# Niccolo-Ajroldi/plainLM

Measured on AMD Instinct MI355X. Metric: tokens/sec fwd+bwd (160M, seq=1024, bf16), higher is better.
Workload: dtype bf16

## Files before the change

plainlm_amd/csrc/attn_causal.hip:

```cpp
#include "plm_device.h"

#include <type_traits>

#include "attn_common.h"

template <int RB>
__device__ __forceinline__ void attn_block2(int T, int nh, int& tile, int& h, int& b) {
  const int ntile = (T + RB - 1) / RB;
  const int nbh = gridDim.x / ntile;
  const int bh = blockIdx.x % nbh;
  tile = blockIdx.x / nbh;
  h = bh % nh;
  b = bh / nh;
}

constexpr int ATTN_DMA_PER_STAGE = 4;
constexpr int ATTN_DMA_STATS = 2;
static_assert(ATTN_DMA_PER_STAGE == 2 * 2, "stage() = two TileDma::issue calls of two instructions each");

#define ATTN_DEFER_LOG2 8.0f
#define PLM_ATTN_TRACE_SETTER plm_dbg_attn_trace_causal
ATTN_TRACE_DECL()
#ifdef PLM_ATTN_ONEPASS_ABLATION
static __device__ float* g_onepass_buf = nullptr;
// ... 68 lines not shown
  f32x16_t o[2][2];
  float mc[2], lsum[2];
#pragma unroll
  for (int qb = 0; qb < 2; ++qb) {
    zero16(o[qb][0]);
    zero16(o[qb][1]);
    mc[qb] = -INFINITY;
    lsum[qb] = 0.f;
  }

  auto soft_pv = [&](int qb_, f32x16_t (&s)[2], const bf16x8_t (&vfr)[2][4], int kv0, auto mask_tag) {
    constexpr bool MASK = decltype(mask_tag)::value;
    const int qb = qb_;
    const int c_hi = r0[qb] + l31 - kv0 - 4 * hi;
    float tmax = -INFINITY;
#pragma unroll
    for (int kb = 0; kb < 2; ++kb)
#pragma unroll
      for (int r = 0; r < 16; ++r) {
        if (MASK) {
          const int c = kb * 32 + (r & 3) + 8 * (r >> 2);
          if (c > c_hi) s[kb][r] = -INFINITY;
        }
        tmax = fmaxf(tmax, s[kb][r]);
      }
    {
      float t_lo, t_hi;
      half_pair(tmax, t_lo, t_hi);
      tmax = fmaxf(t_lo, t_hi);
    }
    const float tm = tmax * c2;
    const bool need = tm > mc[qb] + ATTN_DEFER_LOG2;
    if (__builtin_amdgcn_ballot_w64(need) != 0ull) {
      const float mn = fmaxf(mc[qb], tm);
      const float alpha = fast_exp2(mc[qb] - ((mn == -INFINITY) ? 0.f : mn));
      mc[qb] = mn;
      lsum[qb] *= alpha;
#pragma unroll
      for (int db = 0; db < 2; ++db)
#pragma unroll
        for (int r = 0; r < 16; ++r) o[qb][db][r] *= alpha;
    }
    const float mref = (MASK && mc[qb] == -INFINITY) ? 0.f : mc[qb];
    float ps[4] = {0.f, 0.f, 0.f, 0.f};
    bf16x8_t pf[4];
#pragma unroll
    for (int kb = 0; kb < 2; ++kb)
#pragma unroll
      for (int r = 0; r < 16; ++r) {
        const float p = fast_exp2(__builtin_fmaf(s[kb][r], c2, -mref));
        ps[r & 3] += p;
        pf[kb * 2 + (r >> 3)][r & 7] = f2bf(p);
      }
    lsum[qb] += (ps[0] + ps[1]) + (ps[2] + ps[3]);
#pragma unroll
    for (int db = 0; db < 2; ++db)
#pragma unroll
      for (int sp = 0; sp < 4; ++sp) o[qb][db] = mfma32(vfr[db][sp], pf[sp], o[qb][db]);
  };

  auto compute = [&](int kv0, const char* sK, const char* sV, auto m0_tag, auto m1_tag) {
    constexpr int M0 = decltype(m0_tag)::value, M1 = decltype(m1_tag)::value;
    bf16x8_t kfr[2][4];
#pragma unroll
    for (int kb = 0; kb < 2; ++kb)
#pragma unroll
      for (int ks = 0; ks < 4; ++ks) kfr[kb][ks] = frag_rows(sK, kb * 32 + l31, ks, hi);
    f32x16_t s[2][2];
#pragma unroll
    for (int qb = 0; qb < 2; ++qb) {
      if ((qb == 0 ? M0 : M1) == QB_OFF) continue;
#pragma unroll
      for (int kb = 0; kb < 2; ++kb) {
        zero16(s[qb][kb]);
#pragma unroll
        for (int ks = 0; ks < 4; ++ks) s[qb][kb] = mfma32(kfr[kb][ks], qf[qb][ks], s[qb][kb]);
      }
    }
    __builtin_amdgcn_sched_barrier(0);
    bf16x8_t vfr[2][4];
#pragma unroll
    for (int db = 0; db < 2; ++db)
#pragma unroll
      for (int sp = 0; sp < 4; ++sp) vfr[db][sp] = frag_cols(sV, db, (sp >> 1) * 32 + (sp & 1) * 16 + 4 * hi, lane);
    if (M0 == QB_UM) soft_pv(0, s[0], vfr, kv0, std::false_type{});
    if (M0 == QB_MASK) soft_pv(0, s[0], vfr, kv0, std::true_type{});
    if (M1 == QB_UM) soft_pv(1, s[1], vfr, kv0, std::false_type{});
    if (M1 == QB_MASK) soft_pv(1, s[1], vfr, kv0, std::true_type{});
  };

  int i = 0, slot = 0;
  auto run = [&](int jt_end, auto m0_tag, auto m1_tag, bool active) {
    for (; jt_lo + i < jt_end; ++i) {
      const int rem = min(NST - 2, n - 1 - i);
      if (NST >= 4 && rem >= 2) attn_wait_vm<2 * ATTN_DMA_PER_STAGE>();
      else if (NST >= 3 && rem == 1) attn_wait_vm<ATTN_DMA_PER_STAGE>();
      else attn_wait_vm<0>();
      attn_barrier();
      if (i + NST - 1 < n) stage(slot == 0 ? NST - 1 : slot - 1, jt_lo + i + NST - 1);
      if (active) compute((jt_lo + i) * KT, smem + slot * 2 * TILE, smem + slot * 2 * TILE + TILE, m0_tag, m1_tag);
      slot = (slot + 1 == NST) ? 0 : slot + 1;
    }
  };
  using OFF_ = std::integral_constant<int, QB_OFF>;
  using UM_ = std::integral_constant<int, QB_UM>;
  using MK_ = std::integral_constant<int, QB_MASK>;
  const int a0 = min(jt_hi, r0[0] / KT), e0 = min(jt_hi, r0[0] / KT + 1);
  const int a1 = min(jt_hi, r0[1] / KT), e1 = min(jt_hi, r0[1] / KT + 1);
  run(a0, UM_{}, UM_{}, true);
  run(e0, MK_{}, UM_{}, true);
  run(a1, OFF_{}, UM_{}, true);
  run(e1, OFF_{}, MK_{}, true);
  run(jt_hi, OFF_{}, OFF_{}, false);

  const RowStage rs{smem + (n % NST) * 2 * TILE + wave * 4096, lane};
#pragma unroll
  for (int qb = 0; qb < 2; ++qb) {
    const int qrow = r0[qb] + l31;
    float l_lo, l_hi;
    half_pair(lsum[qb], l_lo, l_hi);
    const float ltot = l_lo + l_hi;
    const float inv = 1.f / ltot;
#pragma unroll
    for (int db = 0; db < 2; ++db)
#pragma unroll
      for (int g = 0; g < 4; ++g) {
        bf16x4_t v;
#pragma unroll
        for (int e = 0; e < 4; ++e) v[e] = f2bf(o[qb][db][4 * g + e] * inv);
        rs.put(l31, hi, db * 4 + g, v);
      }
    if (qrow < T && hi == 0) lse[((int64_t)b * nh + h) * T + qrow] = mc[qb] + __builtin_amdgcn_logf(ltot);
    rs.flush(out + (int64_t)b * T * dm, dm, r0[qb], T, h * HD);
  }
}

template <int NST>
__global__ __launch_bounds__(256, 2) void attn_bwd_dq_causal_kernel(const uint16_t* __restrict__ qkv, const uint16_t* __restrict__ out,
                                                              const uint16_t* __restrict__ dout, const float* __restrict__ lse,
                                                              float* __restrict__ delta, const float* __restrict__ rcos,
                                                              const float* __restrict__ rsin, uint16_t* __restrict__ dqkv, int T, int nh,
                                                              float dsign) {
  constexpr int KT = 64;
  constexpr int TILE = KT * 128;
  constexpr int QB = 256;
  __shared__ __attribute__((aligned(1024))) char smem[NST * 2 * TILE];

  int tile_, h, b;
  attn_block2<QB>(T, nh, tile_, h, b);
  const int qt = (T + QB - 1) / QB - 1 - tile_;
  const int dm = nh * HD, ld = 3 * dm;
  const int t = threadIdx.x, lane = t & 63;
  const int wave = __builtin_amdgcn_readfirstlane(t >> 6);
  const int l31 = lane & 31, hi = lane >> 5;
  const int q0 = qt * QB;
  const int r0[2] = {q0 + 32 * wave, q0 + 32 * (7 - wave)};
  const uint16_t* base = qkv + (int64_t)b * T * ld + h * HD;
  const float scale = 0.125f, c2 = scale * LOG2E;

  const int kv_hi = min(T, q0 + QB);
  const int jt_hi = (kv_hi + KT - 1) / KT;
  constexpr int jt_lo = 0;
  const int n = jt_hi;

  TileDma dma;
  dma.init(wave, lane, ld);
  auto stage = [&](int slot, int jt) {
    const int kv0 = jt * KT;
    const uint16_t* src = base + (int64_t)kv0 * ld;
    if (kv0 + KT <= T) {
      dma.issue_full(smem + slot * 2 * TILE, src + dm, wave);
      dma.issue_full(smem + slot * 2 * TILE + TILE, src + 2 * dm, wave);
    } else {
      dma.issue(smem + slot * 2 * TILE, src + dm, ld, T - 1 - kv0, wave);
      dma.issue(smem + slot * 2 * TILE + TILE, src + 2 * dm, ld, T - 1 - kv0, wave);
    }
  };

  if (n > 0) stage(0, jt_lo);

  bf16x8_t qf[2][4], dof[2][4];
  float Lq[2], Dq[2];
#pragma unroll
  for (int qb = 0; qb < 2; ++qb) {
    const int qrow = r0[qb] + l31;
    const bool qvalid = qrow < T;
#pragma unroll
    for (int ks = 0; ks < 4; ++ks) {
      const int d0 = ks * 16 + hi * 8;
      qf[qb][ks] = qvalid ? ld_bf16x8(base + (int64_t)qrow * ld + d0) : zero_bf16x8();
      dof[qb][ks] = qvalid ? ld_bf16x8(dout + ((int64_t)b * T + qrow) * dm + h * HD + d0) : zero_bf16x8();
    }
    Lq[qb] = 0.f;
    float part = 0.f;
    if (qvalid) {
      Lq[qb] = lse[((int64_t)b * nh + h) * T + qrow];
#pragma unroll
      for (int ks = 0; ks < 4; ++ks) {
        const bf16x8_t o8 = ld_bf16x8(out + ((int64_t)b * T + qrow) * dm + h * HD + ks * 16 + hi * 8);
#pragma unroll
        for (int e = 0; e < 8; ++e) part += bf2f(o8[e]) * bf2f(dof[qb][ks][e]);
      }
    }
    float d_lo, d_hi;
    half_pair(part, d_lo, d_hi);
    Dq[qb] = d_lo + d_hi;
  }
#pragma unroll
  for (int qb = 0; qb < 2; ++qb)
    asm volatile("; q/dO fragments resident" ::"v"(qf[qb][0]), "v"(qf[qb][1]), "v"(qf[qb][2]), "v"(qf[qb][3]), "v"(dof[qb][0]), "v"(dof[qb][1]),
                 "v"(dof[qb][2]), "v"(dof[qb][3]), "v"(Lq[qb]), "v"(Dq[qb]));
  asm volatile("s_waitcnt vmcnt(0)" ::: "memory");
#pragma unroll
  for (int i = 1; i < NST - 1; ++i)
    if (i < n) stage(i, jt_lo + i);

  f32x16_t dq[2][2];
#pragma unroll
  for (int qb = 0; qb < 2; ++qb) {
    zero16(dq[qb][0]);
    zero16(dq[qb][1]);
  }

  auto block = [&](int qb_, int kb, const bf16x8_t (&kfr)[4], const bf16x8_t (&vfr)[4], const bf16x8_t (&ktr)[2][2], int kv0, auto mask_tag) {
    constexpr bool MASK = decltype(mask_tag)::value;
    const int qb = qb_;
    const int c_hi = r0[qb] + l31 - kv0 - 4 * hi;
    f32x16_t s, dp;
    zero16(s);
    zero16(dp);
#pragma unroll
    for (int ks = 0; ks < 4; ++ks) {
      s = mfma32(kfr[ks], qf[qb][ks], s);
      dp = mfma32(vfr[ks], dof[qb][ks], dp);
    }
    bf16x8_t dsf[2];
#pragma unroll
    for (int r = 0; r < 16; ++r) {
      float p = fast_exp2(__builtin_fmaf(s[r], c2, -Lq[qb]));
      if (MASK) {
        const int c = kb * 32 + (r & 3) + 8 * (r >> 2);
        p = (c <= c_hi) ? p : 0.f;
      }
      dsf[r >> 3][r & 7] = f2bf(p * (dp[r] - Dq[qb]));
    }
#pragma unroll
    for (int s2 = 0; s2 < 2; ++s2)
#pragma unroll
      for (int db = 0; db < 2; ++db) dq[qb][db] = mfma32(ktr[db][s2], dsf[s2], dq[qb][db]);
  };

  auto compute = [&](int kv0, const char* sK, const char* sV, auto m0_tag, auto m1_tag) {
    constexpr int M0 = decltype(m0_tag)::value, M1 = decltype(m1_tag)::value;
#pragma unroll
    for (int kb = 0; kb < 2; ++kb) {
      __builtin_amdgcn_sched_barrier(0);
      bf16x8_t kfr[4], vfr[4], ktr[2][2];
#pragma unroll
      for (int ks = 0; ks < 4; ++ks) {
        kfr[ks] = frag_rows(sK, kb * 32 + l31, ks, hi);
        vfr[ks] = frag_rows(sV, kb * 32 + l31, ks, hi);
      }
#pragma unroll
      for (int s2 = 0; s2 < 2; ++s2)
#pragma unroll
        for (int db = 0; db < 2; ++db) ktr[db][s2] = frag_cols(sK, db, kb * 32 + s2 * 16 + 4 * hi, lane);
      if (M0 == QB_UM) block(0, kb, kfr, vfr, ktr, kv0, std::false_type{});
      if (M0 == QB_MASK) block(0, kb, kfr, vfr, ktr, kv0, std::true_type{});
      if (M1 == QB_UM) block(1, kb, kfr, vfr, ktr, kv0, std::false_type{});
      if (M1 == QB_MASK) block(1, kb, kfr, vfr, ktr, kv0, std::true_type{});
    }
  };

  int i = 0, slot = 0;
  auto run = [&](int jt_end, auto m0_tag, auto m1_tag, bool active) {
    for (; jt_lo + i < jt_end; ++i) {
      const int rem = min(NST - 2, n - 1 - i);
      if (NST >= 4 && rem >= 2) attn_wait_vm<2 * ATTN_DMA_PER_STAGE>();
      else if (NST >= 3 && rem == 1) attn_wait_vm<ATTN_DMA_PER_STAGE>();
      else attn_wait_vm<0>();
      attn_barrier();
      if (i + NST - 1 < n) stage(slot == 0 ? NST - 1 : slot - 1, jt_lo + i + NST - 1);
      if (active) compute((jt_lo + i) * KT, smem + slot * 2 * TILE, smem + slot * 2 * TILE + TILE, m0_tag, m1_tag);
      slot = (slot + 1 == NST) ? 0 : slot + 1;
    }
  };
  using OFF_ = std::integral_constant<int, QB_OFF>;
  using UM_ = std::integral_constant<int, QB_UM>;
  using MK_ = std::integral_constant<int, QB_MASK>;
  const int a0 = min(jt_hi, r0[0] / KT), e0 = min(jt_hi, r0[0] / KT + 1);
  const int a1 = min(jt_hi, r0[1] / KT), e1 = min(jt_hi, r0[1] / KT + 1);
  run(a0, UM_{}, UM_{}, true);
  run(e0, MK_{}, UM_{}, true);
  run(a1, OFF_{}, UM_{}, true);
  run(e1, OFF_{}, MK_{}, true);
  run(jt_hi, OFF_{}, OFF_{}, false);

  const RowStage rs{smem + (n % NST) * 2 * TILE + wave * 4096, lane};
#pragma unroll
  for (int qb = 0; qb < 2; ++qb) {
    if (r0[qb] + l31 < T && hi == 0) delta[((int64_t)b * nh + h) * T + r0[qb] + l31] = Dq[qb] * dsign;
#pragma unroll
    for (int db = 0; db < 2; ++db)
#pragma unroll
      for (int g = 0; g < 4; ++g) {
        bf16x4_t ov;
#pragma unroll
        for (int e = 0; e < 4; ++e) ov[e] = f2bf(dq[qb][db][4 * g + e] * scale);
        rs.put(l31, hi, db * 4 + g, ov);
      }
    rs.flush_rot(dqkv + (int64_t)b * T * ld, ld, r0[qb], T, h * HD, rcos, rsin);
  }
}

template <int NST, bool DOC>
__device__ __forceinline__ void attn_bwd_dkdv_body(char* smem, const uint16_t* __restrict__ qkv, const uint16_t* __restrict__ dout,
                                                   const float* __restrict__ lse, const float* __restrict__ ndelta,
                                                   const float* __restrict__ rcos, const float* __restrict__ rsin,
                                                   const int32_t* __restrict__ doc_end, uint16_t* __restrict__ dqkv, int T, int nh, int b, int h,
                                                   int kv0, int jq_plan, unsigned long long* trace_t = nullptr) {
  constexpr int QT = 64;
  constexpr int TILE = QT * 128;
  constexpr int STAGE = 2 * TILE + 512;
  constexpr int NQB = 2;
  const int dm = nh * HD, ld = 3 * dm;
  const int t = threadIdx.x, lane = t & 63;
  const int wave = __builtin_amdgcn_readfirstlane(t >> 6);
  const int l31 = lane & 31, hi = lane >> 5;
  constexpr int qoff = 0;
  const int kvw0 = kv0 + 32 * wave;
  const int kvrow = kvw0 + l31;
  const bool kvalid = kvrow < T;
  const uint16_t* base = qkv + (int64_t)b * T * ld + h * HD;
  const uint16_t* dobase = dout + (int64_t)b * T * dm + h * HD;
  const float* lrow = lse + ((int64_t)b * nh + h) * T;
  const float* drow = ndelta + ((int64_t)b * nh + h) * T;
  const float scale = 0.125f, c2 = scale * LOG2E;

  const int nqt = (T + QT - 1) / QT;
  const int jq_lo = kv0 / QT;
  const int jq_hi = DOC ? jq_plan : nqt;
  const int n = jq_hi - jq_lo;

  TileDma dma, dmad;
  dma.init(wave, lane, ld);
  dmad.init(wave, lane, dm);
  auto stage = [&](int slot, int jq) {
    const int qt0 = jq * QT;
    char* dst = smem + slot * STAGE;
    if (qt0 + QT <= T) {
      dma.issue_full(dst, base + (int64_t)qt0 * ld, wave);
      dmad.issue_full(dst + TILE, dobase + (int64_t)qt0 * dm, wave);
    } else {
      dma.issue(dst, base + (int64_t)qt0 * ld, ld, T - 1 - qt0, wave);
      dma.issue(dst + TILE, dobase + (int64_t)qt0 * dm, dm, T - 1 - qt0, wave);
    }
    if (wave == 0 && lane < 16) {
      const int q = min(qt0 + lane * 4, T - 4);
      dma16_asm(lrow + q, dst + 2 * TILE);
      dma16_asm(drow + q, dst + 2 * TILE + 256);
    }
  };
  bf16x8_t kf[4], vf[4];
  int de = T;
  if (DOC) {
    static_assert(!DOC || NST == 3, "the prologue parks the wave's rows in slots 1 and 2");
    if (n > 0) stage(0, jq_lo);
    char* kreg = smem + 1 * STAGE + wave * 4096;
    char* vreg = smem + 2 * STAGE + wave * 4096;
    rows_dma(kreg, base + dm, ld, kvw0, T - 1, lane);
    rows_dma(vreg, base + 2 * dm, ld, kvw0, T - 1, lane);
    de = doc_end[(int64_t)b * T + min(kvrow, T - 1)];
    asm volatile("; row data requested" ::"v"(de));
    asm volatile("s_waitcnt vmcnt(0)" ::: "memory");
#pragma unroll
    for (int ks = 0; ks < 4; ++ks) {
      kf[ks] = rows_frag(kreg, l31, ks, hi);
      vf[ks] = rows_frag(vreg, l31, ks, hi);
    }
    attn_barrier();
    if (n > 1) stage(1, jq_lo + 1);
  } else {
#pragma unroll
    for (int i = 0; i < NST - 1; ++i)
      if (i < n) stage(i, jq_lo + i);
#pragma unroll
    for (int ks = 0; ks < 4; ++ks) {
      const uint16_t* p = base + (int64_t)kvrow * ld + ks * 16 + hi * 8;
      kf[ks] = kvalid ? ld_bf16x8(p + dm) : zero_bf16x8();
      vf[ks] = kvalid ? ld_bf16x8(p + 2 * dm) : zero_bf16x8();
    }
    asm volatile("; k/v fragments resident" ::"v"(kf[0]), "v"(kf[1]), "v"(kf[2]), "v"(kf[3]), "v"(vf[0]), "v"(vf[1]), "v"(vf[2]), "v"(vf[3]));
    asm volatile("s_waitcnt vmcnt(0)" ::: "memory");
  }
  const int de_lo = DOC ? __builtin_amdgcn_readlane(de, 0) : T, de_hi = DOC ? __builtin_amdgcn_readlane(de, 31) : T;

  f32x16_t dk[2], dv[2];
  zero16(dk[0]); zero16(dk[1]); zero16(dv[0]); zero16(dv[1]);

  auto compute = [&](int qt0, const char* sQ, auto mask_tag) {
    constexpr bool MASK = decltype(mask_tag)::value;
    const char* sDO = sQ + TILE;
    const float* sL = reinterpret_cast<const float*>(sQ + 2 * TILE);
    const float* sD = sL + 64;
    const int c_lo = kvrow - qt0 - qoff - 4 * hi, c_end = de - qt0 - qoff - 4 * hi;
#pragma unroll
    for (int qb = 0; qb < NQB; ++qb) {
      __builtin_amdgcn_sched_barrier(0);
      if (MASK && qt0 + qoff + qb * 32 + 31 < kvw0) continue;
      if (DOC && MASK && qt0 + qoff + qb * 32 >= de_hi) continue;
      bf16x8_t qfr[4], dofr[4], dotr[2][2], qtr[2][2];
#pragma unroll
      for (int ks = 0; ks < 4; ++ks) {
        qfr[ks] = frag_rows(sQ, qoff + qb * 32 + l31, ks, hi);
        dofr[ks] = frag_rows(sDO, qoff + qb * 32 + l31, ks, hi);
      }
      f32x4_t L4[4];
      f32x16_t s, dp;
#pragma unroll
      for (int g = 0; g < 4; ++g) {
        const int ql0 = qoff + qb * 32 + 8 * g + 4 * hi;
        L4[g] = *reinterpret_cast<const f32x4_t*>(sL + ql0);
        const f32x4_t nd = *reinterpret_cast<const f32x4_t*>(sD + ql0);
#pragma unroll
        for (int e = 0; e < 4; ++e) dp[4 * g + e] = nd[e];
      }
#pragma unroll
      for (int s2 = 0; s2 < 2; ++s2)
#pragma unroll
        for (int db = 0; db < 2; ++db) {
          dotr[db][s2] = frag_cols(sDO, db, qoff + qb * 32 + s2 * 16 + 4 * hi, lane);
          qtr[db][s2] = frag_cols(sQ, db, qoff + qb * 32 + s2 * 16 + 4 * hi, lane);
        }
      zero16(s);
#pragma unroll
      for (int ks = 0; ks < 4; ++ks) {
        s = mfma32(qfr[ks], kf[ks], s);
        dp = mfma32(dofr[ks], vf[ks], dp);
      }
      bf16x8_t pf[2], dsf[2];
#pragma unroll
      for (int g = 0; g < 4; ++g)
#pragma unroll
        for (int e = 0; e < 4; ++e) {
          const int r = 4 * g + e;
          float p = fast_exp2(__builtin_fmaf(s[r], c2, -L4[g][e]));
          if (MASK) {
            const int c = qb * 32 + 8 * g + e;
            p = ((c >= c_lo) && (c < c_end)) ? p : 0.f;
          }
          const float dsv = p * dp[r];
          pf[r >> 3][r & 7] = f2bf(p);
          dsf[r >> 3][r & 7] = f2bf(dsv);
        }
#pragma unroll
      for (int s2 = 0; s2 < 2; ++s2)
#pragma unroll
        for (int db = 0; db < 2; ++db) {
          dv[db] = mfma32(dotr[db][s2], pf[s2], dv[db]);
          dk[db] = mfma32(qtr[db][s2], dsf[s2], dk[db]);
        }
#ifdef PLM_ATTN_ONEPASS_ABLATION
      if (g_onepass_mode) {
        char* scr = smem + NST * STAGE + wave * 2048;
        *reinterpret_cast<bf16x8_t*>(scr + lane * 32) = dsf[0];
        *reinterpret_cast<bf16x8_t*>(scr + lane * 32 + 16) = dsf[1];
        bf16x8_t at[2];
#pragma unroll
        for (int s2 = 0; s2 < 2; ++s2)
          at[s2] = join_tr(lds_read_tr16(scr + s2 * 1024 + (lane & 15) * 64 + (lane >> 4) * 8), lds_read_tr16(scr + s2 * 1024 + 512 + (lane & 15) * 32 + (lane >> 4) * 8));
        f32x16_t dqp[2];
        zero16(dqp[0]);
        zero16(dqp[1]);
#pragma unroll
        for (int s2 = 0; s2 < 2; ++s2)
#pragma unroll
          for (int db = 0; db < 2; ++db) dqp[db] = mfma32(at[s2], frag_cols(sQ, db, qoff + qb * 32 + s2 * 16 + 4 * hi, lane), dqp[db]);
        if (g_onepass_mode == 2) {
#pragma unroll
          for (int db = 0; db < 2; ++db)
#pragma unroll
            for (int r = 0; r < 16; ++r) {
              const int q = min(qt0 + qb * 32 + mfma32_row(r, hi), T - 1);
              atomicAdd(g_onepass_buf + ((int64_t)b * T + q) * dm + h * HD + db * 32 + l31, dqp[db][r]);
            }
        } else {
          asm volatile("; partial dQ" ::"v"(dqp[0]), "v"(dqp[1]));
        }
      }
#endif
    }
  };

  const bool wave_rows = kvw0 < T;
  const int jq_act = wave_rows ? min(jq_hi, max(jq_lo, kvw0 / QT)) : jq_hi;
  const int jq_m = min(jq_hi, max(jq_act, (kvw0 + 31 + QT - 1) / QT));
  const int jq_u = min(jq_hi, max(jq_m, de_lo / QT));
  const int jq_e = min(jq_hi, max(jq_u, (de_hi + QT - 1) / QT));
#ifdef PLM_ATTN_TRACE
  if (trace_t) trace_t[0] = __builtin_amdgcn_s_memrealtime();
#endif
  int i = 0, slot = 0;
  auto run = [&](int jq_end, auto mask_tag, bool active) {
    for (; jq_lo + i < jq_end; ++i) {
      const int rem = min(NST - 2, n - 1 - i);
      constexpr int W0 = ATTN_DMA_PER_STAGE + ATTN_DMA_STATS;
      if (wave == 0) {
        if (NST >= 4 && rem >= 2) attn_wait_vm<2 * W0>();
        else if (NST >= 3 && rem == 1) attn_wait_vm<W0>();
        else attn_wait_vm<0>();
      } else {
        if (NST >= 4 && rem >= 2) attn_wait_vm<2 * ATTN_DMA_PER_STAGE>();
        else if (NST >= 3 && rem == 1) attn_wait_vm<ATTN_DMA_PER_STAGE>();
        else attn_wait_vm<0>();
      }
      attn_barrier();
      if (i + NST - 1 < n) stage(slot == 0 ? NST - 1 : slot - 1, jq_lo + i + NST - 1);
      if (active) compute((jq_lo + i) * QT, smem + slot * STAGE, mask_tag);
      slot = (slot + 1 == NST) ? 0 : slot + 1;
    }
  };
  run(jq_act, std::true_type{}, false);
  run(jq_m, std::true_type{}, true);
  run(jq_u, std::false_type{}, true);
  run(jq_e, std::true_type{}, true);
  if (DOC) run(jq_hi, std::true_type{}, false);
#ifdef PLM_ATTN_TRACE
  if (trace_t) trace_t[1] = __builtin_amdgcn_s_memrealtime();
#endif

  const RowStage rs{smem + (n % NST) * STAGE + wave * 4096, lane};
#pragma unroll
  for (int db = 0; db < 2; ++db)
#pragma unroll
    for (int g = 0; g < 4; ++g) {
      bf16x4_t ov;
#pragma unroll
      for (int e = 0; e < 4; ++e) ov[e] = f2bf(dv[db][4 * g + e]);
      rs.put(l31, hi, db * 4 + g, ov);
    }
  rs.flush(dqkv + (int64_t)b * T * ld, ld, kvw0, T, 2 * dm + h * HD);
#pragma unroll
  for (int db = 0; db < 2; ++db)
#pragma unroll
    for (int g = 0; g < 4; ++g) {
      bf16x4_t ok;
#pragma unroll
      for (int e = 0; e < 4; ++e) ok[e] = f2bf(dk[db][4 * g + e] * scale);
      rs.put(l31, hi, db * 4 + g, ok);
    }
  rs.flush_rot(dqkv + (int64_t)b * T * ld, ld, kvw0, T, dm + h * HD, rcos, rsin);
}


template <int NST>
__global__ __launch_bounds__(256, 2) void attn_bwd_dkdv_causal_kernel(const uint16_t* __restrict__ qkv, const uint16_t* __restrict__ dout,
                                                                      const float* __restrict__ lse, const float* __restrict__ ndelta,
                                                                      const float* __restrict__ rcos, const float* __restrict__ rsin,
                                                                      uint16_t* __restrict__ dqkv, int T, int nh) {
  __shared__ __attribute__((aligned(1024))) char smem[NST * (2 * 8192 + 512) + ONEPASS_LDS];
  int kt, h, b;
  attn_block2<128>(T, nh, kt, h, b);
  attn_bwd_dkdv_body<NST, false>(smem, qkv, dout, lse, ndelta, rcos, rsin, nullptr, dqkv, T, nh, b, h, kt * 128, 0);
}

template <int NST>
__global__ __launch_bounds__(256, 2) void attn_bwd_dkdv_doc_kernel(const uint16_t* __restrict__ qkv, const uint16_t* __restrict__ dout,
                                                                   const float* __restrict__ lse, const float* __restrict__ ndelta,
                                                                   const float* __restrict__ rcos, const float* __restrict__ rsin,
                                                                   const int32_t* __restrict__ header, const int32_t* __restrict__ doc_end,
                                                                   const int4* __restrict__ items, uint16_t* __restrict__ dqkv, int T, int nh) {
  __shared__ __attribute__((aligned(1024))) char smem[NST * (2 * 8192 + 512) + ONEPASS_LDS];
  ATTN_TRACE_T(tr0);
  const int idx = blockIdx.x / nh, h = blockIdx.x - idx * nh;
  if (idx >= __builtin_amdgcn_readfirstlane(header[0])) return;
  const int4 it = items[idx];
  const int b = __builtin_amdgcn_readfirstlane(it.x), kv0 = __builtin_amdgcn_readfirstlane(it.y), jq_hi = __builtin_amdgcn_readfirstlane(it.z);
  const int kc = __builtin_amdgcn_readfirstlane(it.w);
  (void)kc;
#ifdef PLM_ATTN_TRACE
  unsigned long long tt[2] = {0, 0};
#else
  unsigned long long* tt = nullptr;
#endif
  attn_bwd_dkdv_body<NST, true>(smem, qkv, dout, lse, ndelta, rcos, rsin, doc_end, dqkv, T, nh, b, h, kv0, jq_hi, tt);
  ATTN_TRACE_END(2, idx, kc, tr0, tt[0], tt[1]);
}

void plm_attn_fwd_causal(const uint16_t* qkv, uint16_t* out, float* lse, int64_t B, int64_t T, int64_t nh, hipStream_t s) {
  const dim3 grid((unsigned)(plm_cdiv(T, 256) * nh * B)), block(256);
  hipLaunchKernelGGL((attn_fwd_causal_kernel<4>), grid, block, 0, s, qkv, out, lse, (int)T, (int)nh);
}
void plm_attn_bwd_causal(const uint16_t* qkv, const uint16_t* out, const uint16_t* dout, const float* lse, float* delta, const float* rc,
                         const float* rs, uint16_t* dqkv, int64_t B, int64_t T, int64_t nh, hipStream_t s) {
  const dim3 block(256);
  hipLaunchKernelGGL((attn_bwd_dq_causal_kernel<3>), dim3((unsigned)(plm_cdiv(T, 256) * nh * B)), block, 0, s, qkv, out, dout, lse, delta, rc, rs, dqkv, (int)T, (int)nh, -1.f);
  hipLaunchKernelGGL((attn_bwd_dkdv_causal_kernel<3>), dim3((unsigned)(plm_cdiv(T, 128) * nh * B)), block, 0, s, qkv, dout, lse, delta, rc, rs, dqkv,
                     (int)T, (int)nh);
}
void plm_attn_bwd_dkdv_doc(const uint16_t* qkv, const uint16_t* dout, const float* lse, const float* ndelta, const float* rc, const float* rs,
                           const int32_t* header, const int32_t* doc_end, const int4* items_k, uint16_t* dqkv, int64_t B, int64_t T, int64_t nh,
                           hipStream_t s) {
  hipLaunchKernelGGL((attn_bwd_dkdv_doc_kernel<3>), dim3((unsigned)(doc_plan_cap(B, T) * nh)), dim3(256), 0, s, qkv, dout, lse, ndelta, rc, rs,
                     header, doc_end, items_k, dqkv, (int)T, (int)nh);
}
```

plainlm_amd/csrc/attn_common.h:

```cpp
#pragma once
#include "plm_device.h"

#define HD 64
#define LOG2E 1.4426950408889634f

__device__ __forceinline__ float fast_exp2(float x) { return __builtin_amdgcn_exp2f(x); }

__device__ __forceinline__ int rs_off(int row, int c) {
  const int pp = ((c >> 1) + 2 * ((row >> 1) & 1) + ((row >> 3) & 1)) & 3;
  const int ph = (c & 1) ^ ((row >> 2) & 1);
  return row * 128 + pp * 32 + ph * 16;
}
__device__ __forceinline__ int rs_logical_chunk(int row, int pc) {
  const int cb = ((pc >> 1) - 2 * ((row >> 1) & 1) - ((row >> 3) & 1)) & 3;
  return cb * 2 + ((pc & 1) ^ ((row >> 2) & 1));
}

__device__ __forceinline__ bf16x8_t frag_rows(const char* tile, int row, int ks, int hi) {
  return *reinterpret_cast<const bf16x8_t*>(tile + rs_off(row, ks * 2 + hi));
}
__device__ __forceinline__ bf16x8_t frag_cols(const char* tile, int db, int rbase, int lane) {
  const int ib = (lane >> 4) & 1, t16 = lane & 15;
  const int sub = t16 & 3;
  const int c = (db * 2 + ib) * 2 + (sub >> 1);
  const int row = rbase + (t16 >> 2);
  const char* p0 = tile + rs_off(row, c) + (sub & 1) * 8;
  const char* p1 = tile + rs_off(row + 8, c) + (sub & 1) * 8;
  return join_tr(lds_read_tr16(p0), lds_read_tr16(p1));
}

struct TileDma {
  int row[2], coff[2];
  unsigned boff[2];
  __device__ __forceinline__ void init(int wave, int lane, int64_t ld = 0) {
#pragma unroll
    for (int i = 0; i < 2; ++i) {
      row[i] = (i * 4 + wave) * 8 + (lane >> 3);
      coff[i] = rs_logical_chunk(row[i], lane & 7) * 8;
      boff[i] = (unsigned)((row[i] * ld + coff[i]) * 2);
    }
  }
  __device__ __forceinline__ void issue(char* dst_tile, const uint16_t* src, int64_t ld, int last_row, int wave, int row0 = 0) const {
#pragma unroll
    for (int i = 0; i < 2; ++i)
      dma16_asm(src + (int64_t)min(row0 + row[i], last_row) * ld + coff[i], dst_tile + (i * 4 + wave) * 1024);
  }
  __device__ __forceinline__ void issue_full(char* dst_tile, const uint16_t* src, int wave) const {
#pragma unroll
    for (int i = 0; i < 2; ++i) dma16_saddr_asm(src, boff[i], dst_tile + (i * 4 + wave) * 1024);
  }
};

__device__ __forceinline__ void rows_dma(char* region, const uint16_t* src, int64_t ld, int row0, int last_row, int lane) {
#pragma unroll
  for (int i = 0; i < 4; ++i) {
    const int row = 8 * i + (lane >> 3);
    dma16_asm(src + (int64_t)min(row0 + row, last_row) * ld + rs_logical_chunk(row, lane & 7) * 8, region + i * 1024);
  }
}
__device__ __forceinline__ bf16x8_t rows_frag(const char* region, int l31, int ks, int hi) {
  return *reinterpret_cast<const bf16x8_t*>(region + rs_off(l31, ks * 2 + hi));
}

template <int N>
__device__ __forceinline__ void attn_wait_vm() {
  asm volatile("s_waitcnt vmcnt(%0)" ::"n"(N) : "memory");
}
__device__ __forceinline__ void attn_barrier() { asm volatile("s_waitcnt lgkmcnt(0)\n\ts_barrier" ::: "memory"); }

__device__ __forceinline__ void zero16(f32x16_t& v) {
#pragma unroll
  for (int r = 0; r < 16; ++r) v[r] = 0.f;
}

struct RowStage {
  char* base;
  int lane;
  __device__ __forceinline__ void put(int l31, int hi, int c16, bf16x4_t v) const {
    *reinterpret_cast<bf16x4_t*>(base + l31 * 128 + ((c16 ^ (l31 & 7)) << 4) + hi * 8) = v;
  }
  __device__ __forceinline__ void flush(uint16_t* dst, int64_t ld, int row0, int row_end, int col0) const {
#pragma unroll
    for (int i = 0; i < 4; ++i) {
      const int row = 8 * i + (lane >> 3), c16 = lane & 7;
      const bf16x8_t v = *reinterpret_cast<const bf16x8_t*>(base + row * 128 + ((c16 ^ (row & 7)) << 4));
      if (row0 + row < row_end) st_bf16x8(dst + (int64_t)(row0 + row) * ld + col0 + c16 * 8, v);
    }
  }
  __device__ __forceinline__ void flush_rot(uint16_t* dst, int64_t ld, int row0, int row_end, int col0, const float* __restrict__ rcos,
                                            const float* __restrict__ rsin) const {
    f32x4_t cs[4], sn[4];
#pragma unroll
    for (int i = 0; i < 4; ++i) {
      const int trow = min(row0 + 8 * i + (lane >> 3), row_end - 1);
      cs[i] = *reinterpret_cast<const f32x4_t*>(rcos + trow * (HD / 2) + (lane & 7) * 4);
      sn[i] = *reinterpret_cast<const f32x4_t*>(rsin + trow * (HD / 2) + (lane & 7) * 4);
    }
#pragma unroll
    for (int i = 0; i < 4; ++i) {
      const int row = 8 * i + (lane >> 3), c16 = lane & 7;
      const bf16x8_t v = *reinterpret_cast<const bf16x8_t*>(base + row * 128 + ((c16 ^ (row & 7)) << 4));
      if (row0 + row < row_end) st_bf16x8(dst + (int64_t)(row0 + row) * ld + col0 + c16 * 8, rope8(v, cs[i], sn[i], -1.f));
    }
  }
};


struct DocPlan {
  const int32_t* header;
  const int32_t* doc_end;
  const int4* items_q;
  const int4* items_k;
};
constexpr int DOC_KIND_SHIFT = 30;
__host__ __device__ __forceinline__ int64_t doc_plan_tiles(int64_t B, int64_t T) { return B * ((T + 127) / 128); }
__host__ __device__ __forceinline__ int64_t doc_plan_cap(int64_t B, int64_t T) { return doc_plan_tiles(B, T) + doc_plan_tiles(B, T) / 4; }
__host__ __device__ __forceinline__ int64_t doc_plan_pq(int64_t B, int64_t T) { return (8 + B * T + 3) & ~(int64_t)3; }
__host__ __device__ __forceinline__ int64_t doc_plan_ints(int64_t B, int64_t T) { return doc_plan_pq(B, T) + 8 * doc_plan_cap(B, T); }
__host__ __device__ __forceinline__ DocPlan doc_plan_view(const int32_t* plan, int64_t B, int64_t T) {
  DocPlan p;
  p.header = plan;
  p.doc_end = plan + 8;
  p.items_q = reinterpret_cast<const int4*>(plan + doc_plan_pq(B, T));
  p.items_k = p.items_q + doc_plan_cap(B, T);
  return p;
}

#ifdef PLM_ATTN_TRACE
#define ATTN_TRACE_DECL()                                                                    \
  static __device__ unsigned long long* g_attn_trace = nullptr;                               \
  extern "C" int PLM_ATTN_TRACE_SETTER(unsigned long long* buf) {                             \
    return (int)hipMemcpyToSymbol(HIP_SYMBOL(g_attn_trace), &buf, sizeof(buf));               \
  }
#define ATTN_TRACE_T(var) const unsigned long long var = __builtin_amdgcn_s_memrealtime()
#define ATTN_TRACE_END(kid, rank_, cost_, t0, t1, t2)                                                                              \
  if (threadIdx.x == 0 && g_attn_trace) {                                                                                          \
    unsigned long long* r_ = g_attn_trace + ((size_t)(kid) * 65536 + blockIdx.x) * 8;                                             \
    r_[0] = t0; r_[1] = t1; r_[2] = t2; r_[3] = __builtin_amdgcn_s_memrealtime();                                                 \
    r_[4] = __builtin_amdgcn_s_getreg((31 << 11) | 4); r_[5] = __builtin_amdgcn_s_getreg((31 << 11) | 20);                         \
    r_[6] = (unsigned long long)(rank_); r_[7] = (unsigned long long)(cost_);                                                      \
  }
#else
#define ATTN_TRACE_DECL()
#define ATTN_TRACE_T(var)
#define ATTN_TRACE_END(kid, rank_, cost_, t0, t1, t2)
#endif
```

Before: 1.053 million.

## Switch causal attention backward kernels from 32x32 to 16x16 MFMA tiles

Rewrites the dQ and dK/dV causal backward kernels to use 16x16x32 MFMA fragments instead of 32x32 ones, with new LDS fragment loaders and a permlane-based row reduction. The finer granularity lets diagonal-masked blocks skip fully masked 16-row sub-blocks, split by wave parity so half the key block is skipped per wave. This trades fewer wasted MFMAs on the causal diagonal for more instructions and fragment loads per useful FLOP and a different register layout.

```diff
diff --git a/plainlm_amd/csrc/attn_causal.hip b/plainlm_amd/csrc/attn_causal.hip
--- a/plainlm_amd/csrc/attn_causal.hip
+++ b/plainlm_amd/csrc/attn_causal.hip
@@ -244,7 +244,6 @@
   const int dm = nh * HD, ld = 3 * dm;
   const int t = threadIdx.x, lane = t & 63;
   const int wave = __builtin_amdgcn_readfirstlane(t >> 6);
-  const int l31 = lane & 31, hi = lane >> 5;
   const int q0 = qt * QB;
   const int r0[2] = {q0 + 32 * wave, q0 + 32 * (7 - wave)};
   const uint16_t* base = qkv + (int64_t)b * T * ld + h * HD;
@@ -271,100 +270,119 @@
 
   if (n > 0) stage(0, jt_lo);
 
-  bf16x8_t qf[2][4], dof[2][4];
-  float Lq[2], Dq[2];
-#pragma unroll
-  for (int qb = 0; qb < 2; ++qb) {
-    const int qrow = r0[qb] + l31;
+  const int l15 = lane & 15, lg = lane >> 4;
+  bf16x8_t qf[4][2], dof[4][2];
+  float Lq[4], Dq[4];
+#pragma unroll
+  for (int j = 0; j < 4; ++j) {
+    const int qrow = r0[j >> 1] + 16 * (j & 1) + l15;
     const bool qvalid = qrow < T;
 #pragma unroll
-    for (int ks = 0; ks < 4; ++ks) {
-      const int d0 = ks * 16 + hi * 8;
-      qf[qb][ks] = qvalid ? ld_bf16x8(base + (int64_t)qrow * ld + d0) : zero_bf16x8();
-      dof[qb][ks] = qvalid ? ld_bf16x8(dout + ((int64_t)b * T + qrow) * dm + h * HD + d0) : zero_bf16x8();
-    }
-    Lq[qb] = 0.f;
+    for (int kk = 0; kk < 2; ++kk) {
+      const int d0 = kchunk16(kk, lg) * 8;
+      qf[j][kk] = qvalid ? ld_bf16x8(base + (int64_t)qrow * ld + d0) : zero_bf16x8();
+      dof[j][kk] = qvalid ? ld_bf16x8(dout + ((int64_t)b * T + qrow) * dm + h * HD + d0) : zero_bf16x8();
+    }
+    Lq[j] = 0.f;
     float part = 0.f;
     if (qvalid) {
-      Lq[qb] = lse[((int64_t)b * nh + h) * T + qrow];
-#pragma unroll
-      for (int ks = 0; ks < 4; ++ks) {
-        const bf16x8_t o8 = ld_bf16x8(out + ((int64_t)b * T + qrow) * dm + h * HD + ks * 16 + hi * 8);
-#pragma unroll
-        for (int e = 0; e < 8; ++e) part += bf2f(o8[e]) * bf2f(dof[qb][ks][e]);
-      }
-    }
-    float d_lo, d_hi;
-    half_pair(part, d_lo, d_hi);
-    Dq[qb] = d_lo + d_hi;
+      Lq[j] = lse[((int64_t)b * nh + h) * T + qrow];
+#pragma unroll
+      for (int kk = 0; kk < 2; ++kk) {
+        const bf16x8_t o8 = ld_bf16x8(out + ((int64_t)b * T + qrow) * dm + h * HD + kchunk16(kk, lg) * 8);
+#pragma unroll
+        for (int e = 0; e < 8; ++e) part += bf2f(o8[e]) * bf2f(dof[j][kk][e]);
+      }
+    }
+    Dq[j] = sum_groups16(part);
   }
 #pragma unroll
-  for (int qb = 0; qb < 2; ++qb)
-    asm volatile("; q/dO fragments resident" ::"v"(qf[qb][0]), "v"(qf[qb][1]), "v"(qf[qb][2]), "v"(qf[qb][3]), "v"(dof[qb][0]), "v"(dof[qb][1]),
-                 "v"(dof[qb][2]), "v"(dof[qb][3]), "v"(Lq[qb]), "v"(Dq[qb]));
+  for (int j = 0; j < 4; ++j)
+    asm volatile("; q/dO fragments resident" ::"v"(qf[j][0]), "v"(qf[j][1]), "v"(dof[j][0]), "v"(dof[j][1]), "v"(Lq[j]), "v"(Dq[j]));
   asm volatile("s_waitcnt vmcnt(0)" ::: "memory");
 #pragma unroll
   for (int i = 1; i < NST - 1; ++i)
     if (i < n) stage(i, jt_lo + i);
 
-  f32x16_t dq[2][2];
-#pragma unroll
-  for (int qb = 0; qb < 2; ++qb) {
-    zero16(dq[qb][0]);
-    zero16(dq[qb][1]);
-  }
-
-  auto block = [&](int qb_, int kb, const bf16x8_t (&kfr)[4], const bf16x8_t (&vfr)[4], const bf16x8_t (&ktr)[2][2], int kv0, auto mask_tag) {
-    constexpr bool MASK = decltype(mask_tag)::value;
-    const int qb = qb_;
-    const int c_hi = r0[qb] + l31 - kv0 - 4 * hi;
-    f32x16_t s, dp;
-    zero16(s);
-    zero16(dp);
-#pragma unroll
-    for (int ks = 0; ks < 4; ++ks) {
-      s = mfma32(kfr[ks], qf[qb][ks], s);
-      dp = mfma32(vfr[ks], dof[qb][ks], dp);
-    }
-    bf16x8_t dsf[2];
-#pragma unroll
-    for (int r = 0; r < 16; ++r) {
-      float p = fast_exp2(__builtin_fmaf(s[r], c2, -Lq[qb]));
-      if (MASK) {
-        const int c = kb * 32 + (r & 3) + 8 * (r >> 2);
-        p = (c <= c_hi) ? p : 0.f;
-      }
-      dsf[r >> 3][r & 7] = f2bf(p * (dp[r] - Dq[qb]));
-    }
-#pragma unroll
-    for (int s2 = 0; s2 < 2; ++s2)
-#pragma unroll
-      for (int db = 0; db < 2; ++db) dq[qb][db] = mfma32(ktr[db][s2], dsf[s2], dq[qb][db]);
-  };
-
-  auto compute = [&](int kv0, const char* sK, const char* sV, auto m0_tag, auto m1_tag) {
+  f32x4_t dq[4][4];
+#pragma unroll
+  for (int j = 0; j < 4; ++j)
+#pragma unroll
+    for (int db = 0; db < 4; ++db) dq[j][db] = f32x4_t{0.f, 0.f, 0.f, 0.f};
+
+  const int dmask = l15 - koff16(lg);
+
+  auto group = [&](auto j_tag, const bf16x8_t (&kfr)[2][2], const bf16x8_t (&vfr)[2][2], const bf16x8_t (&ktr)[4], auto live_tag, auto ma_tag) {
+    constexpr int J = decltype(j_tag)::value, LIVE = decltype(live_tag)::value, MA = decltype(ma_tag)::value;
+    bf16x8_t dsf;
+#pragma unroll
+    for (int a = 0; a < 2; ++a) {
+      if (a < LIVE) {
+        f32x4_t s = {0.f, 0.f, 0.f, 0.f}, dp = {0.f, 0.f, 0.f, 0.f};
+#pragma unroll
+        for (int kk = 0; kk < 2; ++kk) {
+          s = mfma16(kfr[a][kk], qf[J][kk], s);
+          dp = mfma16(vfr[a][kk], dof[J][kk], dp);
+        }
+#pragma unroll
+        for (int r = 0; r < 4; ++r) {
+          float p = fast_exp2(__builtin_fmaf(s[r], c2, -Lq[J]));
+          if (a == MA) p = (r <= dmask) ? p : 0.f;
+          dsf[4 * a + r] = f2bf(p * (dp[r] - Dq[J]));
+        }
+      } else {
+#pragma unroll
+        for (int r = 0; r < 4; ++r) dsf[4 * a + r] = f2bf(0.f);
+      }
+    }
+#pragma unroll
+    for (int db = 0; db < 4; ++db) dq[J][db] = mfma16(ktr[db], dsf, dq[J][db]);
+  };
+
+  using G0_ = std::integral_constant<int, 0>;
+  using G1_ = std::integral_constant<int, 1>;
+  using G2_ = std::integral_constant<int, 2>;
+  using GN_ = std::integral_constant<int, -1>;
+  auto compute = [&](const char* sK, const char* sV, auto m0_tag, auto m1_tag, bool kd0, bool kd1) {
     constexpr int M0 = decltype(m0_tag)::value, M1 = decltype(m1_tag)::value;
-#pragma unroll
-    for (int kb = 0; kb < 2; ++kb) {
+    auto key_block = [&](auto kb_tag) {
+      constexpr int KB = decltype(kb_tag)::value;
+      if (KB == 1 && M0 != QB_UM && M1 != QB_UM && !(M0 == QB_MASK ? kd0 : kd1)) return;
       __builtin_amdgcn_sched_barrier(0);
-      bf16x8_t kfr[4], vfr[4], ktr[2][2];
-#pragma unroll
-      for (int ks = 0; ks < 4; ++ks) {
-        kfr[ks] = frag_rows(sK, kb * 32 + l31, ks, hi);
-        vfr[ks] = frag_rows(sV, kb * 32 + l31, ks, hi);
-      }
-#pragma unroll
-      for (int s2 = 0; s2 < 2; ++s2)
-#pragma unroll
-        for (int db = 0; db < 2; ++db) ktr[db][s2] = frag_cols(sK, db, kb * 32 + s2 * 16 + 4 * hi, lane);
-      if (M0 == QB_UM) block(0, kb, kfr, vfr, ktr, kv0, std::false_type{});
-      if (M0 == QB_MASK) block(0, kb, kfr, vfr, ktr, kv0, std::true_type{});
-      if (M1 == QB_UM) block(1, kb, kfr, vfr, ktr, kv0, std::false_type{});
-      if (M1 == QB_MASK) block(1, kb, kfr, vfr, ktr, kv0, std::true_type{});
-    }
+      bf16x8_t kfr[2][2], vfr[2][2], ktr[4];
+#pragma unroll
+      for (int a = 0; a < 2; ++a)
+#pragma unroll
+        for (int kk = 0; kk < 2; ++kk) {
+          kfr[a][kk] = frag_rows16(sK, KB * 32 + 16 * a, kk, lane);
+          vfr[a][kk] = frag_rows16(sV, KB * 32 + 16 * a, kk, lane);
+        }
+#pragma unroll
+      for (int db = 0; db < 4; ++db) ktr[db] = frag_cols16(sK, db, KB * 32, lane);
+      auto row_block = [&](auto ja_tag, auto jb_tag, auto m_tag, bool kd) {
+        constexpr int M = decltype(m_tag)::value;
+        if constexpr (M == QB_UM) {
+          group(ja_tag, kfr, vfr, ktr, G2_{}, GN_{});
+          group(jb_tag, kfr, vfr, ktr, G2_{}, GN_{});
+        } else if constexpr (M == QB_MASK) {
+          if (kd == (KB == 1)) {
+            group(ja_tag, kfr, vfr, ktr, G1_{}, G0_{});
+            group(jb_tag, kfr, vfr, ktr, G2_{}, G1_{});
+          } else if (KB == 0) {
+            group(ja_tag, kfr, vfr, ktr, G2_{}, GN_{});
+            group(jb_tag, kfr, vfr, ktr, G2_{}, GN_{});
+          }
+        }
+      };
+      row_block(G0_{}, G1_{}, m0_tag, kd0);
+      row_block(G2_{}, std::integral_constant<int, 3>{}, m1_tag, kd1);
+    };
+    key_block(G0_{});
+    key_block(G1_{});
   };
 
   int i = 0, slot = 0;
+  const bool kd0 = (wave & 1) != 0, kd1 = !kd0;
   auto run = [&](int jt_end, auto m0_tag, auto m1_tag, bool active) {
     for (; jt_lo + i < jt_end; ++i) {
       const int rem = min(NST - 2, n - 1 - i);
@@ -373,7 +391,7 @@
       else attn_wait_vm<0>();
       attn_barrier();
       if (i + NST - 1 < n) stage(slot == 0 ? NST - 1 : slot - 1, jt_lo + i + NST - 1);
-      if (active) compute((jt_lo + i) * KT, smem + slot * 2 * TILE, smem + slot * 2 * TILE + TILE, m0_tag, m1_tag);
+      if (active) compute(smem + slot * 2 * TILE, smem + slot * 2 * TILE + TILE, m0_tag, m1_tag, kd0, kd1);
       slot = (slot + 1 == NST) ? 0 : slot + 1;
     }
   };
@@ -391,16 +409,18 @@
   const RowStage rs{smem + (n % NST) * 2 * TILE + wave * 4096, lane};
 #pragma unroll
   for (int qb = 0; qb < 2; ++qb) {
-    if (r0[qb] + l31 < T && hi == 0) delta[((int64_t)b * nh + h) * T + r0[qb] + l31] = Dq[qb] * dsign;
-#pragma unroll
-    for (int db = 0; db < 2; ++db)
-#pragma unroll
-      for (int g = 0; g < 4; ++g) {
+#pragma unroll
+    for (int half = 0; half < 2; ++half) {
+      const int j = 2 * qb + half;
+      if (r0[qb] + 16 * half + l15 < T && lg == 0) delta[((int64_t)b * nh + h) * T + r0[qb] + 16 * half + l15] = Dq[j] * dsign;
+#pragma unroll
+      for (int db = 0; db < 4; ++db) {
         bf16x4_t ov;
 #pragma unroll
-        for (int e = 0; e < 4; ++e) ov[e] = f2bf(dq[qb][db][4 * g + e] * scale);
-        rs.put(l31, hi, db * 4 + g, ov);
-      }
+        for (int e = 0; e < 4; ++e) ov[e] = f2bf(dq[j][db][e] * scale);
+        rs.put(16 * half + l15, lg & 1, 2 * db + (lg >> 1), ov);
+      }
+    }
     rs.flush_rot(dqkv + (int64_t)b * T * ld, ld, r0[qb], T, h * HD, rcos, rsin);
   }
 }
@@ -418,11 +438,9 @@
   const int dm = nh * HD, ld = 3 * dm;
   const int t = threadIdx.x, lane = t & 63;
   const int wave = __builtin_amdgcn_readfirstlane(t >> 6);
-  const int l31 = lane & 31, hi = lane >> 5;
-  constexpr int qoff = 0;
+  const int l15 = lane & 15, lg = lane >> 4;
   const int kvw0 = kv0 + 32 * wave;
-  const int kvrow = kvw0 + l31;
-  const bool kvalid = kvrow < T;
+  const int kvrow[2] = {kvw0 + l15, kvw0 + 16 + l15};
   const uint16_t* base = qkv + (int64_t)b * T * ld + h * HD;
   const uint16_t* dobase = dout + (int64_t)b * T * dm + h * HD;
   const float* lrow = lse + ((int64_t)b * nh + h) * T;
@@ -453,8 +471,8 @@
       dma16_asm(drow + q, dst + 2 * TILE + 256);
     }
   };
-  bf16x8_t kf[4], vf[4];
-  int de = T;
+  bf16x8_t kf[2][2], vf[2][2];
+  int de[2] = {T, T};
   if (DOC) {
     static_assert(!DOC || NST == 3, "the prologue parks the wave's rows in slots 1 and 2");
     if (n > 0) stage(0, jq_lo);
@@ -462,14 +480,17 @@
     char* vreg = smem + 2 * STAGE + wave * 4096;
     rows_dma(kreg, base + dm, ld, kvw0, T - 1, lane);
     rows_dma(vreg, base + 2 * dm, ld, kvw0, T - 1, lane);
-    de = doc_end[(int64_t)b * T + min(kvrow, T - 1)];
-    asm volatile("; row data requested" ::"v"(de));
+#pragma unroll
+    for (int jk = 0; jk < 2; ++jk) de[jk] = doc_end[(int64_t)b * T + min(kvrow[jk], T - 1)];
+    asm volatile("; row data requested" ::"v"(de[0]), "v"(de[1]));
     asm volatile("s_waitcnt vmcnt(0)" ::: "memory");
 #pragma unroll
-    for (int ks = 0; ks < 4; ++ks) {
-      kf[ks] = rows_frag(kreg, l31, ks, hi);
-      vf[ks] = rows_frag(vreg, l31, ks, hi);
-    }
+    for (int jk = 0; jk < 2; ++jk)
+#pragma unroll
+      for (int kk = 0; kk < 2; ++kk) {
+        kf[jk][kk] = rows_frag16(kreg, 16 * jk + l15, kk, lg);
+        vf[jk][kk] = rows_frag16(vreg, 16 * jk + l15, kk, lg);
+      }
     attn_barrier();
     if (n > 1) stage(1, jq_lo + 1);
   } else {
@@ -477,86 +498,103 @@
     for (int i = 0; i < NST - 1; ++i)
       if (i < n) stage(i, jq_lo + i);
 #pragma unroll
-    for (int ks = 0; ks < 4; ++ks) {
-      const uint16_t* p = base + (int64_t)kvrow * ld + ks * 16 + hi * 8;
-      kf[ks] = kvalid ? ld_bf16x8(p + dm) : zero_bf16x8();
-      vf[ks] = kvalid ? ld_bf16x8(p + 2 * dm) : zero_bf16x8();
-    }
-    asm volatile("; k/v fragments resident" ::"v"(kf[0]), "v"(kf[1]), "v"(kf[2]), "v"(kf[3]), "v"(vf[0]), "v"(vf[1]), "v"(vf[2]), "v"(vf[3]));
+    for (int jk = 0; jk < 2; ++jk)
+#pragma unroll
+      for (int kk = 0; kk < 2; ++kk) {
+        const uint16_t* p = base + (int64_t)kvrow[jk] * ld + kchunk16(kk, lg) * 8;
+        kf[jk][kk] = kvrow[jk] < T ? ld_bf16x8(p + dm) : zero_bf16x8();
+        vf[jk][kk] = kvrow[jk] < T ? ld_bf16x8(p + 2 * dm) : zero_bf16x8();
+      }
+    asm volatile("; k/v fragments resident" ::"v"(kf[0][0]), "v"(kf[0][1]), "v"(kf[1][0]), "v"(kf[1][1]), "v"(vf[0][0]), "v"(vf[0][1]), "v"(vf[1][0]), "v"(vf[1][1]));
     asm volatile("s_waitcnt vmcnt(0)" ::: "memory");
   }
-  const int de_lo = DOC ? __builtin_amdgcn_readlane(de, 0) : T, de_hi = DOC ? __builtin_amdgcn_readlane(de, 31) : T;
-
-  f32x16_t dk[2], dv[2];
-  zero16(dk[0]); zero16(dk[1]); zero16(dv[0]); zero16(dv[1]);
+  const int de_lo = DOC ? __builtin_amdgcn_readlane(de[0], 0) : T, de_hi = DOC ? __builtin_amdgcn_readlane(de[1], 15) : T;
+
+  f32x4_t dk[2][4], dv[2][4];
+#pragma unroll
+  for (int jk = 0; jk < 2; ++jk)
+#pragma unroll
+    for (int db = 0; db < 4; ++db) dk[jk][db] = dv[jk][db] = f32x4_t{0.f, 0.f, 0.f, 0.f};
 
   auto compute = [&](int qt0, const char* sQ, auto mask_tag) {
-    constexpr bool MASK = decltype(mask_tag)::value;
+    constexpr int MASK = decltype(mask_tag)::value;
     const char* sDO = sQ + TILE;
     const float* sL = reinterpret_cast<const float*>(sQ + 2 * TILE);
     const float* sD = sL + 64;
-    const int c_lo = kvrow - qt0 - qoff - 4 * hi, c_end = de - qt0 - qoff - 4 * hi;
+    int c_lo[2], c_end[2];
+#pragma unroll
+    for (int jk = 0; jk < 2; ++jk) {
+      c_lo[jk] = kvrow[jk] - qt0 - koff16(lg);
+      c_end[jk] = de[jk] - qt0 - koff16(lg);
+    }
+    const bool diag1 = MASK == 2 && qt0 + 32 == kvw0;
 #pragma unroll
     for (int qb = 0; qb < NQB; ++qb) {
       __builtin_amdgcn_sched_barrier(0);
-      if (MASK && qt0 + qoff + qb * 32 + 31 < kvw0) continue;
-      if (DOC && MASK && qt0 + qoff + qb * 32 >= de_hi) continue;
-      bf16x8_t qfr[4], dofr[4], dotr[2][2], qtr[2][2];
-#pragma unroll
-      for (int ks = 0; ks < 4; ++ks) {
-        qfr[ks] = frag_rows(sQ, qoff + qb * 32 + l31, ks, hi);
-        dofr[ks] = frag_rows(sDO, qoff + qb * 32 + l31, ks, hi);
-      }
-      f32x4_t L4[4];
-      f32x16_t s, dp;
-#pragma unroll
-      for (int g = 0; g < 4; ++g) {
-        const int ql0 = qoff + qb * 32 + 8 * g + 4 * hi;
-        L4[g] = *reinterpret_cast<const f32x4_t*>(sL + ql0);
-        const f32x4_t nd = *reinterpret_cast<const f32x4_t*>(sD + ql0);
-#pragma unroll
-        for (int e = 0; e < 4; ++e) dp[4 * g + e] = nd[e];
-      }
-#pragma unroll
-      for (int s2 = 0; s2 < 2; ++s2)
-#pragma unroll
-        for (int db = 0; db < 2; ++db) {
-          dotr[db][s2] = frag_cols(sDO, db, qoff + qb * 32 + s2 * 16 + 4 * hi, lane);
-          qtr[db][s2] = frag_cols(sQ, db, qoff + qb * 32 + s2 * 16 + 4 * hi, lane);
-        }
-      zero16(s);
-#pragma unroll
-      for (int ks = 0; ks < 4; ++ks) {
-        s = mfma32(qfr[ks], kf[ks], s);
-        dp = mfma32(dofr[ks], vf[ks], dp);
-      }
-      bf16x8_t pf[2], dsf[2];
-#pragma unroll
-      for (int g = 0; g < 4; ++g)
-#pragma unroll
-        for (int e = 0; e < 4; ++e) {
-          const int r = 4 * g + e;
-          float p = fast_exp2(__builtin_fmaf(s[r], c2, -L4[g][e]));
-          if (MASK) {
-            const int c = qb * 32 + 8 * g + e;
-            p = ((c >= c_lo) && (c < c_end)) ? p : 0.f;
+      if (MASK && qt0 + qb * 32 + 31 < kvw0) continue;
+      if (DOC && MASK && qt0 + qb * 32 >= de_hi) continue;
+      bf16x8_t qfr[2][2], dofr[2][2], dotr[4], qtr[4];
+      f32x4_t L4[2], nd[2];
+#pragma unroll
+      for (int a = 0; a < 2; ++a) {
+#pragma unroll
+        for (int kk = 0; kk < 2; ++kk) {
+          qfr[a][kk] = frag_rows16(sQ, qb * 32 + 16 * a, kk, lane);
+          dofr[a][kk] = frag_rows16(sDO, qb * 32 + 16 * a, kk, lane);
+        }
+        L4[a] = *reinterpret_cast<const f32x4_t*>(sL + qb * 32 + 16 * a + koff16(lg));
+        nd[a] = *reinterpret_cast<const f32x4_t*>(sD + qb * 32 + 16 * a + koff16(lg));
+      }
+#pragma unroll
+      for (int db = 0; db < 4; ++db) {
+        dotr[db] = frag_cols16(sDO, db, qb * 32, lane);
+        qtr[db] = frag_cols16(sQ, db, qb * 32, lane);
+      }
+      auto key_group = [&](int jk_, auto dead0_tag) {
+        constexpr bool DEAD0 = decltype(dead0_tag)::value;
+        const int jk = jk_;
+        bf16x8_t pf, dsf;
+#pragma unroll
+        for (int a = 0; a < 2; ++a) {
+          if (DEAD0 && a == 0) {
+#pragma unroll
+            for (int r = 0; r < 4; ++r) pf[r] = dsf[r] = f2bf(0.f);
+            continue;
           }
-          const float dsv = p * dp[r];
-          pf[r >> 3][r & 7] = f2bf(p);
-          dsf[r >> 3][r & 7] = f2bf(dsv);
-        }
-#pragma unroll
-      for (int s2 = 0; s2 < 2; ++s2)
-#pragma unroll
-        for (int db = 0; db < 2; ++db) {
-          dv[db] = mfma32(dotr[db][s2], pf[s2], dv[db]);
-          dk[db] = mfma32(qtr[db][s2], dsf[s2], dk[db]);
-        }
+          f32x4_t s = {0.f, 0.f, 0.f, 0.f}, dp = nd[a];
+#pragma unroll
+          for (int kk = 0; kk < 2; ++kk) {
+            s = mfma16(qfr[a][kk], kf[jk][kk], s);
+            dp = mfma16(dofr[a][kk], vf[jk][kk], dp);
+          }
+#pragma unroll
+          for (int r = 0; r < 4; ++r) {
+            float p = fast_exp2(__builtin_fmaf(s[r], c2, -L4[a][r]));
+            if (MASK) {
+              const int c = qb * 32 + 16 * a + r;
+              p = ((c >= c_lo[jk]) && (c < c_end[jk])) ? p : 0.f;
+            }
+            pf[4 * a + r] = f2bf(p);
+            dsf[4 * a + r] = f2bf(p * dp[r]);
+          }
+        }
+#pragma unroll
+        for (int db = 0; db < 4; ++db) {
+          dv[jk][db] = mfma16(dotr[db], pf, dv[jk][db]);
+          dk[jk][db] = mfma16(qtr[db], dsf, dk[jk][db]);
+        }
+        return dsf;
+      };
+      bf16x8_t dsk[2];
+      dsk[0] = key_group(0, std::false_type{});
+      if (MASK == 2 && (qb == 1) == diag1) dsk[1] = key_group(1, std::true_type{});
+      else dsk[1] = key_group(1, std::false_type{});
+      (void)dsk;
 #ifdef PLM_ATTN_ONEPASS_ABLATION
       if (g_onepass_mode) {
         char* scr = smem + NST * STAGE + wave * 2048;
-        *reinterpret_cast<bf16x8_t*>(scr + lane * 32) = dsf[0];
-        *reinterpret_cast<bf16x8_t*>(scr + lane * 32 + 16) = dsf[1];
+        *reinterpret_cast<bf16x8_t*>(scr + lane * 32) = dsk[0];
+        *reinterpret_cast<bf16x8_t*>(scr + lane * 32 + 16) = dsk[1];
         bf16x8_t at[2];
 #pragma unroll
         for (int s2 = 0; s2 < 2; ++s2)
@@ -567,14 +605,14 @@
 #pragma unroll
         for (int s2 = 0; s2 < 2; ++s2)
 #pragma unroll
-          for (int db = 0; db < 2; ++db) dqp[db] = mfma32(at[s2], frag_cols(sQ, db, qoff + qb * 32 + s2 * 16 + 4 * hi, lane), dqp[db]);
+          for (int db = 0; db < 2; ++db) dqp[db] = mfma32(at[s2], frag_cols(sQ, db, qb * 32 + s2 * 16 + 4 * (lane >> 5), lane), dqp[db]);
         if (g_onepass_mode == 2) {
 #pragma unroll
           for (int db = 0; db < 2; ++db)
 #pragma unroll
             for (int r = 0; r < 16; ++r) {
-              const int q = min(qt0 + qb * 32 + mfma32_row(r, hi), T - 1);
-              atomicAdd(g_onepass_buf + ((int64_t)b * T + q) * dm + h * HD + db * 32 + l31, dqp[db][r]);
+              const int q = min(qt0 + qb * 32 + mfma32_row(r, lane >> 5), T - 1);
+              atomicAdd(g_onepass_buf + ((int64_t)b * T + q) * dm + h * HD + db * 32 + (lane & 31), dqp[db][r]);
             }
         } else {
           asm volatile("; partial dQ" ::"v"(dqp[0]), "v"(dqp[1]));
@@ -612,34 +650,37 @@
       slot = (slot + 1 == NST) ? 0 : slot + 1;
     }
   };
-  run(jq_act, std::true_type{}, false);
-  run(jq_m, std::true_type{}, true);
-  run(jq_u, std::false_type{}, true);
-  run(jq_e, std::true_type{}, true);
-  if (DOC) run(jq_hi, std::true_type{}, false);
+  using M0_ = std::integral_constant<int, 0>;
+  using M1_ = std::integral_constant<int, 1>;
+  using MD_ = std::integral_constant<int, DOC ? 1 : 2>;
+  run(jq_act, M1_{}, false);
+  run(jq_m, MD_{}, true);
+  run(jq_u, M0_{}, true);
+  run(jq_e, M1_{}, true);
+  if (DOC) run(jq_hi, M1_{}, false);
 #ifdef PLM_ATTN_TRACE
   if (trace_t) trace_t[1] = __builtin_amdgcn_s_memrealtime();
 #endif
 
   const RowStage rs{smem + (n % NST) * STAGE + wave * 4096, lane};
 #pragma unroll
-  for (int db = 0; db < 2; ++db)
-#pragma unroll
-    for (int g = 0; g < 4; ++g) {
+  for (int jk = 0; jk < 2; ++jk)
+#pragma unroll
+    for (int db = 0; db < 4; ++db) {
       bf16x4_t ov;
 #pragma unroll
-      for (int e = 0; e < 4; ++e) ov[e] = f2bf(dv[db][4 * g + e]);
-      rs.put(l31, hi, db * 4 + g, ov);
+      for (int e = 0; e < 4; ++e) ov[e] = f2bf(dv[jk][db][e]);
+      rs.put(16 * jk + l15, lg & 1, 2 * db + (lg >> 1), ov);
     }
   rs.flush(dqkv + (int64_t)b * T * ld, ld, kvw0, T, 2 * dm + h * HD);
 #pragma unroll
-  for (int db = 0; db < 2; ++db)
-#pragma unroll
-    for (int g = 0; g < 4; ++g) {
+  for (int jk = 0; jk < 2; ++jk)
+#pragma unroll
+    for (int db = 0; db < 4; ++db) {
       bf16x4_t ok;
 #pragma unroll
-      for (int e = 0; e < 4; ++e) ok[e] = f2bf(dk[db][4 * g + e] * scale);
-      rs.put(l31, hi, db * 4 + g, ok);
+      for (int e = 0; e < 4; ++e) ok[e] = f2bf(dk[jk][db][e] * scale);
+      rs.put(16 * jk + l15, lg & 1, 2 * db + (lg >> 1), ok);
     }
   rs.flush_rot(dqkv + (int64_t)b * T * ld, ld, kvw0, T, dm + h * HD, rcos, rsin);
 }
diff --git a/plainlm_amd/csrc/attn_common.h b/plainlm_amd/csrc/attn_common.h
--- a/plainlm_amd/csrc/attn_common.h
+++ b/plainlm_amd/csrc/attn_common.h
@@ -27,6 +27,28 @@
   const char* p0 = tile + rs_off(row, c) + (sub & 1) * 8;
   const char* p1 = tile + rs_off(row + 8, c) + (sub & 1) * 8;
   return join_tr(lds_read_tr16(p0), lds_read_tr16(p1));
+}
+
+__device__ __forceinline__ constexpr int kchunk16(int kk, int g) { return 4 * (g & 1) + 2 * (g >> 1) + kk; }
+__device__ __forceinline__ constexpr int koff16(int g) { return 8 * (g & 1) + 4 * (g >> 1); }
+__device__ __forceinline__ constexpr int blk16_row(int i) { return (i & 3) + koff16(i >> 2); }
+__device__ __forceinline__ bf16x8_t frag_rows16(const char* tile, int row0, int kk, int lane) {
+  return *reinterpret_cast<const bf16x8_t*>(tile + rs_off(row0 + blk16_row(lane & 15), kchunk16(kk, lane >> 4)));
+}
+__device__ __forceinline__ bf16x8_t frag_cols16(const char* tile, int db16, int row0, int lane) {
+  const int t16 = lane & 15, sub = t16 & 3;
+  const int c = db16 * 2 + (sub >> 1);
+  const int row = row0 + koff16(lane >> 4) + (t16 >> 2);
+  const char* p0 = tile + rs_off(row, c) + (sub & 1) * 8;
+  const char* p1 = tile + rs_off(row + 16, c) + (sub & 1) * 8;
+  return join_tr(lds_read_tr16(p0), lds_read_tr16(p1));
+}
+__device__ __forceinline__ float sum_groups16(float v) {
+  float a = v, b = v;
+  asm volatile("s_nop 1\n\tv_permlane16_swap_b32 %0, %1" : "+v"(a), "+v"(b));
+  float lo, hi;
+  half_pair(a + b, lo, hi);
+  return lo + hi;
 }
 
 struct TileDma {
@@ -60,6 +82,9 @@
 }
 __device__ __forceinline__ bf16x8_t rows_frag(const char* region, int l31, int ks, int hi) {
   return *reinterpret_cast<const bf16x8_t*>(region + rs_off(l31, ks * 2 + hi));
+}
+__device__ __forceinline__ bf16x8_t rows_frag16(const char* region, int row, int kk, int g) {
+  return *reinterpret_cast<const bf16x8_t*>(region + rs_off(row, kchunk16(kk, g)));
 }
 
 template <int N>
```

Result: no change. 1.057 million, median of 6 (+0.4%).
